# HKUST-Aerial-Robotics/ESVO

Measured on AMD Instinct MI355X. Metric: mapped events/sec (stereo TS raster + block matching + LM depth refinement + fusion), events resident in HBM before the timed region; exactly K ticks between two synchronisations, i.e. including the fill and the drain of the two-deep tick pipeline (`sustained`: the same workload over 1600 ticks), higher is better.
Workload: dtype f64

## Files before the change

esvo_amd/csrc/api_core.hip:

```cpp
#include "context.hpp"

namespace esvo_host {
thread_local std::string g_create_error;
}

namespace {

void invert3x3(const double* P, double* Kinv, double* Kinv_t) {
  const double a = P[0], b = P[1], cc = P[2], d = P[4], e = P[5], f = P[6], g = P[8], hh = P[9], i = P[10];
  const double det = a * (e * i - f * hh) - b * (d * i - f * g) + cc * (d * hh - e * g);
  const double id = 1.0 / det;
  Kinv[0] = (e * i - f * hh) * id; Kinv[1] = (cc * hh - b * i) * id; Kinv[2] = (b * f - cc * e) * id;
  Kinv[3] = (f * g - d * i) * id;  Kinv[4] = (a * i - cc * g) * id;  Kinv[5] = (cc * d - a * f) * id;
  Kinv[6] = (d * hh - e * g) * id; Kinv[7] = (b * g - a * hh) * id;  Kinv[8] = (a * e - b * d) * id;
  for (int r = 0; r < 3; ++r) Kinv_t[r] = (Kinv[r * 3 + 0] * P[3] + Kinv[r * 3 + 1] * P[7]) + Kinv[r * 3 + 2] * P[11];
}

int validate_params(const esvo_params_t* p, std::string& why) {
  if (p->ls_norm != ESVO_LSNORM_TDIST && p->ls_norm != ESVO_LSNORM_L2) { why = "LSnorm must be Tdist or l2 (DepthProblemSolver.cpp:121-131 exits on anything else)"; return ESVO_ERR_UNSUPPORTED; }
  if (p->bm_step < 1) { why = "BM_step must be >= 1"; return ESVO_ERR_INVALID_ARG; }
  if (p->patch_size_x < 1 || p->patch_size_x > 64 || p->patch_size_y < 1 || p->patch_size_y > 40) { why = "patch size must be within 1..64 x 1..40"; return ESVO_ERR_UNSUPPORTED; }
  if (p->median_blur_kernel_size < 0 || p->median_blur_kernel_size > 3) { why = "median_blur_kernel_size must be 0..3 (kernel 2k + 1)"; return ESVO_ERR_UNSUPPORTED; }
  if (p->max_event_queue_len < 0 || p->max_event_queue_len > TSQ_LMAX) { why = "max_event_queue_len must be 0 (one stamp per pixel) or 1..32"; return ESVO_ERR_UNSUPPORTED; }
  if (p->bm_max_disparity < p->bm_min_disparity || p->bm_min_disparity < 0) { why = "bad disparity range"; return ESVO_ERR_INVALID_ARG; }
// ... 194 lines not shown
  h->ring_cap = (u64)std::max<int64_t>(params->event_ring_capacity, 1024);
  for (int cam = 0; cam < 2; ++cam) CK(dalloc(&h->d_ring[cam], h->ring_cap));
  h->max_poses = (u32)std::max(params->max_poses_per_tick, 2);
  CK(dalloc(&h->d_pose_T2[0], (size_t)h->max_poses * 17));
  CK(dalloc(&h->d_pose_T2[1], (size_t)h->max_poses * 17));
  h->d_pose_T = h->d_pose_T2[0];
  h->max_ev = (u32)std::max(params->max_events_per_tick, params->process_event_num) + 1u;
  if (h->max_ev > 4000000u) { g_create_error = "max_events_per_tick too large (scan limit 4M)"; esvo_destroy(h); return ESVO_ERR_CAPACITY; }
  if (npx > 4000000u) { g_create_error = "image too large (scan limit 4M pixels)"; esvo_destroy(h); return ESVO_ERR_CAPACITY; }
  const size_t E = h->max_ev;
  CK(dalloc(&h->d_tick_ev, E));
  CK(dalloc(&h->d_match_slots, E));
  CK(dalloc(&h->d_match_flags, E));
  CK(dalloc(&h->d_match_prefix, E));
  CK(dalloc(&h->d_matches2[0], E));
  CK(dalloc(&h->d_matches2[1], E));
  h->d_matches = h->d_matches2[0];
  if (E >= LM_SPLIT_MIN_EVENTS) {
    CK(dalloc(&h->d_lm_fvec0, E * 7 * 16));
    CK(dalloc(&h->d_lm_fnorm0, E));
    CK(dalloc(&h->d_lm_meta, E));
    CK(dalloc(&h->d_lm_order, E));
    CK(dalloc(&h->d_lm_hist, 2 * 32 * 64));
    CK(hipMemset(h->d_lm_hist, 0, sizeof(u32) * 2 * 32 * 64));
  }
  if (E > LM_TWO_QUEUES_MAX_EVENTS) {
    for (int k = 0; k < 2; ++k) {
      CK(dalloc(&h->d_lm_pix_order2[k], E));
      CK(dalloc(&h->d_lm_sort_rows[k], E));
    }
    CK(dalloc(&h->d_lm_sort_hist, voxel_hist_words(E)));
    if (const char* eo = esvo_dev_switch("ESVO_LM_ORDER")) h->lm_order_on = std::atoi(eo) != 0;
  }
  CK(dalloc(&h->d_clk, 2 * clk_words(h->max_ev)));
  CK(hipMemset(h->d_clk, 0, sizeof(u64) * 2 * clk_words(h->max_ev)));
  if (const char* ec = esvo_dev_switch("ESVO_CLK_PROBE")) h->clk_probe = std::atoi(ec) != 0;
  {
    int khz = 0;
    if (hipDeviceGetAttribute(&khz, hipDeviceAttributeWallClockRate, device) != hipSuccess || khz <= 0) khz = 100000;
    h->stats.clk_ref_khz = (uint32_t)khz;
  }
  for (int k = 0; k < 2; ++k) {
    CK(dalloc(&h->d_pt_slots2[k], E));
    CK(dalloc(&h->d_pt_flags2[k], E));
    CK(dalloc(&h->d_pt_prefix2[k], E));
    CK(dalloc(&h->d_scan_tmp_l2[k], scan_scratch_elems(std::max(E, npx)) + 8));
  }
  h->d_pt_slots = h->d_pt_slots2[0]; h->d_pt_flags = h->d_pt_flags2[0]; h->d_pt_prefix = h->d_pt_prefix2[0];
  h->d_scan_tmp_l = h->d_scan_tmp_l2[0];
  CK(dalloc(&h->d_pts_tmp, E));
  CK(dalloc(&h->d_stage[0], E));
  CK(dalloc(&h->d_stage[1], E));
  CK(dalloc(&h->d_counters2[0], CNT_ROW));
  CK(dalloc(&h->d_counters2[1], CNT_ROW));
  CK(hipMemset(h->d_counters2[0], 0, sizeof(u32) * CNT_ROW));
  CK(hipMemset(h->d_counters2[1], 0, sizeof(u32) * CNT_ROW));
  h->d_counters = h->d_counters2[0];
  CK(hipHostMalloc(reinterpret_cast<void**>(&h->h_counters), sizeof(u32) * CNT_ROW * 2));
  std::memset(h->h_counters, 0, sizeof(u32) * CNT_ROW * 2);
  CK(hipHostMalloc(reinterpret_cast<void**>(&h->h_pin), sizeof(double) * 2 * ((size_t)h->max_poses * 17 + 16)));
  CK(dalloc(&h->d_scan_tmp, scan_scratch_elems(std::max(E, npx)) + 8));
  CK(dalloc(&h->d_scan_tmp_b, scan_scratch_elems(std::max(E, npx)) + 8));
  CK(dalloc(&h->d_cnt_b, CNTB_ROW));
  CK(hipMemset(h->d_cnt_b, 0, sizeof(u32) * CNTB_ROW));
  CK(hipHostMalloc(reinterpret_cast<void**>(&h->h_cnt_b), sizeof(u32) * CNTB_ROW * CNTB_ROWS));
  std::memset(h->h_cnt_b, 0, sizeof(u32) * CNTB_ROW * CNTB_ROWS);
// ... 50 lines not shown
  CK(dalloc(&h->d_export_cell, npx));
  for (int i = 0; i < EV_N; ++i) CK(hipEventCreate(&h->evt[i]));
  if (h->tl_on) { CK(hipEventCreate(&h->tl_ref)); CK(hipEventRecord(h->tl_ref, h->stream)); CK(hipEventSynchronize(h->tl_ref)); }
  h->evt_ok = true;
  CK(hipEventCreateWithFlags(&h->evt_trk_read, hipEventDisableTiming));
  for (int cam = 0; cam < 2; ++cam) CK(hipEventCreateWithFlags(&h->evt_ingest[cam], hipEventDisableTiming));
  CK(hipHostMalloc(reinterpret_cast<void**>(&h->h_pose_pool), sizeof(double) * 16 * (size_t)h->max_poses * esvo_context::POSE_POOL));
  for (int i = 0; i < esvo_context::POSE_POOL; ++i) CK(hipEventCreate(&h->pool_evt[i]));
  h->pool_ok = true;
  for (int i = 0; i < 16; ++i) h->T_world_obs[i] = h->T_world_frame[i] = (i % 5 == 0) ? 1.0 : 0.0;
#undef CK
  *out = h;
  return ESVO_OK;
}

int esvo_destroy(esvo_handle h) {
  if (!h) return ESVO_OK;
  hipSetDevice(h->device);
  if (h->stream) hipStreamSynchronize(h->stream);
  if (h->stream_l) hipStreamSynchronize(h->stream_l);
  if (h->stream_l1) hipStreamSynchronize(h->stream_l1);
  if (h->stream_b) hipStreamSynchronize(h->stream_b);
  comm_release(h);
  em_release(h);
  gpc_release(h);
  void* ptrs[] = {h->d_lut, h->d_mask, h->d_fixmap[0], h->d_fixmap[1], h->d_sae[0], h->d_sae[1], h->d_raw, h->d_raw1, h->d_fwd_lut[0], h->d_fwd_lut[1], h->d_fwd_off[0], h->d_fwd_off[1],
                  h->d_fwd_src[0], h->d_fwd_src[1], h->d_fwd_val, h->d_ts[0],
                  h->d_ts[1], h->d_ring[0], h->d_ring[1], h->d_obs2[0][0], h->d_obs2[0][1], h->d_obs2[1][0], h->d_obs2[1][1], h->d_obs_tmp,
                  h->d_pose_T2[0], h->d_pose_T2[1], h->d_scan_tmp_b, h->d_cnt_b, h->d_tick_ev, h->d_match_slots, h->d_match_flags, h->d_match_prefix,
                  h->d_matches2[0], h->d_matches2[1], h->d_scan_tmp_l2[0], h->d_scan_tmp_l2[1], h->d_pt_slots2[0], h->d_pt_slots2[1], h->d_pt_flags2[0], h->d_pt_flags2[1], h->d_pt_prefix2[0], h->d_pt_prefix2[1], h->d_pts_tmp, h->d_stage[0], h->d_stage[1], h->d_counters2[0], h->d_counters2[1], h->d_scan_tmp,
                  h->d_win, h->d_frame_pose_T, h->d_fr_table, h->d_prop, h->d_tile_pts, h->d_tile_count, h->d_over_pts,
                  h->d_cell_count, h->d_cell_offset, h->d_cell_list, h->d_fuse_ctr, h->d_rec_ids, h->d_map, h->d_map2, h->d_owner_max, h->d_owner_min, h->d_exp_flags,
                  h->d_exp_prefix, h->d_export, h->d_export_cell, h->d_reg_ab, h->d_reg_cd, h->d_tsq[0], h->d_tsq[1], h->d_tsq_tcount, h->d_tsq_tlist, h->d_tsq_over, h->d_tsq_over_count, h->d_own_w, h->d_lkeep, h->d_codes, h->d_codes_send, h->d_codes_all, h->d_pts_send, h->d_pts_all, h->d_rank_kept,
                  h->d_sel, h->d_evmap, h->d_lm_fvec0, h->d_lm_fnorm0, h->d_lm_meta, h->d_lm_order, h->d_lm_hist, h->d_lm_pix_order2[0], h->d_lm_pix_order2[1], h->d_lm_sort_rows[0], h->d_lm_sort_rows[1], h->d_lm_sort_hist, h->d_clk, h->d_ring_gidx, h->d_halo_viol, h->d_dn_flags, h->d_merge_a, h->d_merge_b, h->d_merge_plan, h->d_tsq_dup};
  for (void* p : ptrs) if (p) hipFree(p);
  if (h->h_counters) hipHostFree(h->h_counters);
  if (h->h_cnt_b) hipHostFree(h->h_cnt_b);
  if (h->h_pin) hipHostFree(h->h_pin);
  if (h->h_fr_table) hipHostFree(h->h_fr_table);
  if (h->evt_ok) for (int i = 0; i < EV_N; ++i) hipEventDestroy(h->evt[i]);
  if (h->pool_ok) for (int i = 0; i < esvo_context::POSE_POOL; ++i) hipEventDestroy(h->pool_evt[i]);
  if (h->h_pose_pool) hipHostFree(h->h_pose_pool);
  if (h->h_trk_ne) hipHostFree(h->h_trk_ne);
  if (h->h_trk_solve) hipHostFree(h->h_trk_solve);
  if (h->h_trk_xyz) hipHostFree(h->h_trk_xyz);
  release_routing(h);
  for (int cam = 0; cam < 2; ++cam) if (h->d_wire[cam]) hipFree(h->d_wire[cam]);
  if (h->evt_trk_read) hipEventDestroy(h->evt_trk_read);
  for (void* q : {(void*)h->d_cloud_xyz[0], (void*)h->d_cloud_xyz[1], (void*)h->d_cloud_ids, (void*)h->d_cloud_scan, (void*)h->d_cloud_cnt}) if (q) hipFree(q);
  if (h->h_cloud_cnt) hipHostFree(h->h_cloud_cnt);
  for (int k = 0; k < 2; ++k) {
    if (h->evt_cloud_built[k]) hipEventDestroy(h->evt_cloud_built[k]);
    if (h->evt_cloud_read[k]) hipEventDestroy(h->evt_cloud_read[k]);
  }
  if (h->tl_ref) hipEventDestroy(h->tl_ref);
  for (int cam = 0; cam < 2; ++cam) if (h->evt_ingest[cam]) hipEventDestroy(h->evt_ingest[cam]);
  for (void* q : {(void*)h->d_viz_bgr, (void*)h->d_viz_jet, (void*)h->d_viz_owner}) if (q) hipFree(q);
  for (void* q : {(void*)h->sgm.sobL, (void*)h->sgm.rawL, (void*)h->sgm.sobR, (void*)h->sgm.rawR, (void*)h->sgm.vol[0], (void*)h->sgm.vol[1],
                  (void*)h->sgm.vol[2], (void*)h->sgm.vol[3], (void*)h->sgm.vol[4], (void*)h->sgm.vol[5], (void*)h->sgm.d1, (void*)h->sgm.d1b,
                  (void*)h->sgm.d2key, (void*)h->d_sgm_img[0], (void*)h->d_sgm_img[1], (void*)h->d_sgm_disp, (void*)h->d_sgm_pair, (void*)h->d_sgm_T})
    if (q) hipFree(q);
  for (hipEvent_t e : h->evt_sgm) if (e) hipEventDestroy(e);
  if (h->own_stream && h->stream) hipStreamDestroy(h->stream);
  if (h->stream_b) hipStreamDestroy(h->stream_b);
  if (h->stream_l) { hipStreamSynchronize(h->stream_l); hipStreamDestroy(h->stream_l); }
  if (h->stream_l1) { hipStreamSynchronize(h->stream_l1); hipStreamDestroy(h->stream_l1); }
  if (h->stream_t) { hipStreamSynchronize(h->stream_t); hipStreamDestroy(h->stream_t); }
// ... 240 lines not shown
```

esvo_amd/csrc/api_dev.hip:

```cpp
#include <vector>

#include "context.hpp"
#include "fdiv.hpp"

namespace {
using esvo::u32;

constexpr size_t GUARD_WORDS = 64;
constexpr size_t GUARD_BYTES = GUARD_WORDS * sizeof(u32);
constexpr u32 GUARD_PATTERN = 0xA55AC33Cu;

struct GBuf {
  uint8_t* base = nullptr;
  size_t bytes = 0;
  bool pinned = false;
  GBuf() = default;
  GBuf(const GBuf&) = delete;
  GBuf& operator=(const GBuf&) = delete;
  ~GBuf() {
    if (!base) return;
    if (pinned) hipHostFree(base);
    else hipFree(base);
  }
  hipError_t make(size_t n, const void* init, bool pin = false) {
// ... 336 lines not shown
    hipLaunchKernelGGL(debug_recip_kernel, dim3(fdiv_blocks(n)), dim3(256), 0, st.s, d_b.ptr<double>(), n, d_m.ptr<double>(),
                       d_r.ptr<double>());
  DEV_RUN_DONE();
  HIPCHK(d_m.finish(y_make, &bad));
  HIPCHK(d_r.finish(y_refined, &bad));
  DEV_RETURN();
}

int esvo_debug_sqrt_moderate(const double* x, size_t n, double* out) {
  if (n && (!x || !out)) return ESVO_ERR_INVALID_ARG;
  DEV_BEGIN();
  GBuf d_x, d_out;
  HIPCHK(d_x.make(n * 8, x));
  HIPCHK(d_out.make(n * 8, out));
  if (n) hipLaunchKernelGGL(debug_sqrt_kernel, dim3(fdiv_blocks(n)), dim3(256), 0, st.s, d_x.ptr<double>(), n, d_out.ptr<double>());
  DEV_RUN_DONE();
  HIPCHK(d_out.finish(out, &bad));
  DEV_RETURN();
}

int esvo_debug_fuse_cell_counts(esvo_handle h, uint32_t* out, size_t n) {
  if (!h || !out) return ESVO_ERR_INVALID_ARG;
  API_LOCK(h);
  if (n != (size_t)h->W * (size_t)h->H) FAIL(ESVO_ERR_INVALID_ARG, "esvo_debug_fuse_cell_counts: width x height words are expected");
  HIPCHK(hipSetDevice(h->device));
  int rc = flush_pending_tick(h);
  if (rc) return rc;
  rc = drain_lm_and_back(h);
  if (rc) return rc;
  HIPCHK(hipMemcpy(out, h->d_cell_count, sizeof(u32) * n, hipMemcpyDeviceToHost));
  return ESVO_OK;
}

}
```

esvo_amd/csrc/api_map.hip:

```cpp
#include "context.hpp"

namespace esvo_host {

u64 lower_bound_sec(const esvo_context* h, int cam, double t) {
  const auto& v = h->ts_host[cam];
  size_t lo = 0, hi = v.size();
  while (lo < hi) {
    size_t mid = (lo + hi) / 2;
    if (ns_to_sec(v[mid]) < t) lo = mid + 1; else hi = mid;
  }
  return h->ring_base[cam] + lo;
}
u64 ros_time_from_sec(double t) {
  long long sec64 = (long long)std::floor(t);
  u32 sec = (u32)sec64;
  u32 nsec = (u32)std::round((t - sec) * 1e9);
  sec += (nsec / 1000000000ul);
  nsec %= 1000000000ul;
  return (u64)sec * 1000000000ull + nsec;
}

int upload_poses(esvo_context* h, const uint64_t* pose_t_ns, const double* pose_T, size_t m, u32* d_zero_row) {
  if (m > h->max_poses) FAIL(ESVO_ERR_CAPACITY, "pose table larger than max_poses_per_tick");
  h->pin_slot ^= 1;
  double* pin = h->h_pin + (size_t)h->pin_slot * ((size_t)h->max_poses * 17 + 16);
  double* T = pin;
  double* sec = pin + 16 * m;
  for (size_t i = 0; i < m; ++i) sec[i] = ns_to_sec(pose_t_ns[i]);
  std::memcpy(T, pose_T, sizeof(double) * 16 * m);
  h->h_pose_T.assign(pose_T, pose_T + 16 * m);
  h->n_pose = (u32)m;
  h->pose_buf ^= 1;
  h->d_pose_T = h->d_pose_T2[h->pose_buf];
  HIPCHK(hipStreamWaitEvent(h->stream, h->evt[EV_POSE + h->pose_buf * EV_BACK_STRIDE], 0));
  h->d_pose_sec = h->d_pose_T + 16 * m;
  launch_upload_words(T, h->d_pose_T, sizeof(double) * 17 * m, h->stream, d_zero_row, CNT_ROW);
  return ESVO_OK;
}

int run_bm(esvo_context* h, const esvo_event_t* d_ev, u64 first, u64 cap, int reverse, u32 n, const u32* sel) {
  BmArgs a;
  a.ev = d_ev; a.n = n; a.ev_first = first; a.ev_cap = cap; a.ev_reverse = reverse; a.sel = sel;
  a.tsL = h->d_obs[0]; a.tsR = h->d_obs[1];
  a.lut = h->d_lut; a.mask = h->d_mask;
  a.pose_sec = h->d_pose_sec; a.n_pose = h->n_pose;
  a.out_slots = h->d_match_slots; a.out_flags = h->d_match_flags;
  a.fail_counters = h->d_counters;
  if (h->stage_events_on) hipEventRecord(h->evt[EV_BM0 + h->fpar * EV_FRONT_STRIDE], h->stream);
  launch_bm_match(a, h->dp, h->stream);
  if (h->stage_events_on) hipEventRecord(h->evt[EV_BM1 + h->fpar * EV_FRONT_STRIDE], h->stream);
  HIPCHK(hipGetLastError());
  return ESVO_OK;
}
int run_order_matches(esvo_context* h, u32 n, bool local, bool by_index) {
  if (scan_compact_is_small(n)) {
    by_index = by_index && !local;
    launch_scan_compact_matches_small(h->d_match_flags, h->d_match_prefix, h->d_counters + (local ? CNT_OWN_MATCHES : CNT_MATCHES), n, h->d_match_slots,
                                      by_index ? nullptr : h->d_matches, (local || by_index) ? h->d_own_w : nullptr, h->stream);
  } else {
    launch_exclusive_scan_u32(h->d_match_flags, h->d_match_prefix, h->d_counters + (local ? CNT_OWN_MATCHES : CNT_MATCHES), h->d_scan_tmp, n, h->stream);
    launch_compact_matches(h->d_match_slots, h->d_match_flags, h->d_match_prefix, n, h->d_matches, local ? h->d_own_w : nullptr,
                           h->stream);
  }
  if (h->stage_events_on) hipEventRecord(h->evt[EV_S1 + h->fpar * EV_FRONT_STRIDE], h->stream);
  HIPCHK(hipGetLastError());
  return ESVO_OK;
}
int run_match(esvo_context* h, const esvo_event_t* d_ev, u64 first, u64 cap, int reverse, u32 n) {
  int rc = run_bm(h, d_ev, first, cap, reverse, n);
  if (rc) return rc;
  return run_order_matches(h, n, false);
}

void switch_front_parity(esvo_context* h) {
  h->fpar ^= 1;
  h->d_matches = h->d_matches2[h->fpar];
  h->d_counters = h->d_counters2[h->fpar];
  h->d_pt_slots = h->d_pt_slots2[h->fpar]; h->d_pt_flags = h->d_pt_flags2[h->fpar]; h->d_pt_prefix = h->d_pt_prefix2[h->fpar];
  h->d_scan_tmp_l = h->d_scan_tmp_l2[h->fpar];
}
static int lm_pair_policy(esvo_context* h, u32 n_events) {
  if (n_events == 0 || n_events > esvo::LM_PAIR_MAX_EVENTS || h->prm.ls_norm == ESVO_LSNORM_L2) return -1;
// ... 576 lines not shown
```

esvo_amd/csrc/common.hpp:

```cpp
#pragma once

#include <hip/hip_runtime.h>
#include <stdint.h>

#include "../../include/esvo_hip.h"

#define ESVO_WAVE 64

#include <cstdlib>
#include <cstring>
inline const char* esvo_dev_switch(const char* name) {
  const char* on = std::getenv("ESVO_DEV_SWITCHES");
  return (on && std::strcmp(on, "1") == 0) ? std::getenv(name) : nullptr;
}

namespace esvo {

typedef unsigned long long u64;
typedef unsigned int u32;

struct CamConst {
  double P[12];
  double Kinv[9];
  double Kinv_t[3];
// ... 166 lines not shown
                              uint8_t* d_raw, uint8_t* d_out, int W, int H, u64 t_ns, double decay_sec, int ignore_polarity,
                              int median_k, hipStream_t s);
void launch_gaussian5_pair(const uint8_t* in0, const uint8_t* in1, uint8_t* out0, uint8_t* out1, int W, int H, hipStream_t s,
                           int row0 = 0, int row1 = -1);
void launch_denoise_flags(const esvo_event_t* ring, u64 first, u64 cap, u32 n, uint8_t* evmap, u32* flags, int W, int H,
                          hipStream_t s);
void launch_denoise_select(const u32* flags, const u32* prefix, u32 n, u32* sel, hipStream_t s);
void launch_denoise_bits_routed(const esvo_event_t* ring, u64 first, u64 cap, u32 n_loc, const u32* gidx, u32 g_first, u32 n, uint8_t* evmap,
                                int W, int H, int band_y0, int band_y1, u32* bits, hipStream_t s);
void launch_denoise_bits_unpack(const u32* blocks, u32 block_words, u32 N, u32 n, u32* flags, hipStream_t s);

struct BmArgs {
  const esvo_event_t* ev;
  u32 n;
  u64 ev_first;
  u64 ev_cap;
  int ev_reverse;
  const u32* sel;
  const uint8_t* tsL;
  const uint8_t* tsR;
  const float2* lut;
  const uint8_t* mask;
  const double* pose_sec;
  u32 n_pose;
  esvo_match_t* out_slots;
  u32* out_flags;
  u32* fail_counters;
  const u32* gidx = nullptr;
  u32 g_first = 0;
  u32 n_loc = 0;
  const u32* keep_flags = nullptr;
  const u32* keep_prefix = nullptr;
  u32 n_raw = 0;
};
void launch_bm_match(const BmArgs& a, const DevParams& p, hipStream_t s);
void launch_compact_matches(const esvo_match_t* slots, const u32* flags, const u32* prefix, u32 n,
                            esvo_match_t* out, u32* slot_of, hipStream_t s);
void launch_matches_to_points(const esvo_match_t* m, const u32* n_ptr, u32 max_n, esvo_depth_point_t* out, const DevParams& p,
                              hipStream_t s);

struct TrackRef { double T[16]; };
struct TrackPose { double T[16]; double Jc[6]; };
#define TRK_NE_MAX_POSES 4
struct TrackPoseSet { TrackPose p[TRK_NE_MAX_POSES]; };
struct TrackArgs {
  const double* pts;
  const uint8_t* neg;
  const int16_t* du;
  const int16_t* dv;
  const uint8_t* mask;
  double P[12];
  int W, H;
};
void launch_track_images(const uint8_t* blurred, uint8_t* neg, int16_t* du, int16_t* dv, int W, int H, hipStream_t s);
void launch_track_reference(const float* xyz, u32 n, const TrackRef& r, double* pts, hipStream_t s);
void launch_track_reference_gather(const float* cloud_xyz, const u32* order, u32 n, const TrackRef& r, double* pts, hipStream_t s);
void launch_track_residuals(const TrackArgs& a, const TrackPose& pose, u32 offset, u32 count, int huber, double thr, double* fvec,
                            hipStream_t s);
void launch_track_jacobian(const TrackArgs& a, const TrackPose& pose, u32 offset, u32 count, double* fjac, hipStream_t s);
#define TRK_NE_THREADS 256
#define TRK_NE_TERMS 28
void launch_track_normal(const TrackArgs& a, const TrackPoseSet& poses, int n_poses, u32 offset, u32 count, int huber, double thr,
                         double* out28_per_pose, hipStream_t s);
#define TRK_SOLVE_MAX_ITERATIONS 64
#define TRK_SOLVE_THREADS 1024
struct TrackSolveArgs {
  double R0[9], t0[3];
  double huber_threshold, damping;
// ... 152 lines not shown
```

esvo_amd/csrc/context.hpp:

```cpp
#pragma once
#include <algorithm>
#include <array>
#include <atomic>
#include <chrono>
#include <cmath>
#include <cstdio>
#include <cstdlib>
#include <cstring>
#include <deque>
#include <mutex>
#include <string>
#include <vector>

#include "common.hpp"

using namespace esvo;

enum { EV_SC0 = 0, EV_SC1, EV_R1, EV_SC0b, EV_SC1b, EV_R1b, EV_FRAME,
       EV_T0, EV_BM0, EV_BM1, EV_S1, EV_LM0, EV_LM1, EV_S2, EV_CNT, EV_STG, EV_A1, EV_T0b, EV_BM0b, EV_BM1b, EV_S1b, EV_LM0b, EV_LM1b, EV_S2b, EV_CNTb, EV_STGb, EV_A1b,
       EV_FU0, EV_FU1, EV_CL1, EV_RG1, EV_POSE, EV_FU0b, EV_FU1b, EV_CL1b, EV_RG1b, EV_POSEb, EV_N };
constexpr int EV_BACK_STRIDE = EV_FU0b - EV_FU0;
constexpr int EV_FRONT_STRIDE = EV_T0b - EV_T0;
constexpr int EV_TS_STRIDE = EV_SC0b - EV_SC0;

// ... 90 lines not shown
  bool ingest_pending[2] = {false, false};

  uint8_t* d_obs[2] = {nullptr, nullptr};
  uint8_t* d_obs_tmp = nullptr;
  double T_world_obs[16];
  u64 obs_t_ns = 0;
  bool obs_set = false;

  double* d_pose_sec = nullptr;
  double* d_pose_T = nullptr;
  double* d_pose_T2[2] = {nullptr, nullptr};
  int pose_buf = 0;
  std::vector<double> h_pose_T;
  double* h_pin = nullptr;
  int pin_slot = 0;
  bool stats_pending = false;
  u32 n_pose = 0;

  u32 max_ev = 0;
  esvo_event_t* d_tick_ev = nullptr;
  esvo_match_t* d_match_slots = nullptr;
  u32* d_match_flags = nullptr;
  u32* d_match_prefix = nullptr;
  esvo_match_t* d_matches = nullptr;
  double* d_lm_fvec0 = nullptr;
  double* d_lm_fnorm0 = nullptr;
  u32* d_lm_meta = nullptr;
  u32* d_lm_order = nullptr;
  u32* d_lm_hist = nullptr;
  u32* d_lm_pix_order2[2] = {nullptr, nullptr};
  u64* d_lm_sort_rows[2] = {nullptr, nullptr};
  u32* d_lm_sort_hist = nullptr;
  bool lm_order_on = true;
  u64* d_clk = nullptr;
  bool clk_probe = true;
  DevPoint* d_pt_slots = nullptr;
  u32* d_pt_flags = nullptr;
  u32* d_pt_prefix = nullptr;
  DevPoint* d_pt_slots2[2] = {nullptr, nullptr};
  u32* d_pt_flags2[2] = {nullptr, nullptr};
  u32* d_pt_prefix2[2] = {nullptr, nullptr};
  DevPoint* d_pts_tmp = nullptr;
  DevPoint* d_stage[2] = {nullptr, nullptr};
  u32* d_counters = nullptr;
  u32* h_counters = nullptr;
  u32* d_scan_tmp = nullptr;
  u32* d_cnt_b = nullptr;
  u32* h_cnt_b = nullptr;
  u32* d_scan_tmp_b = nullptr;

  DevPoint* d_win = nullptr;
  u32 win_cap = 0;
  std::deque<FrameRec> frames;
  u32 n_pose_slots = 0;
  std::vector<char> slot_used;
  double* d_frame_pose_T = nullptr;
  u32 max_poses = 0;
  u32* d_fr_table = nullptr;
  u32* h_fr_table = nullptr;
  u32 max_frames = 0;
  size_t n_window_frames = 0;

  DevPoint* d_prop = nullptr;
  u32* d_tile_count = nullptr;
  uint2* d_tile_pts = nullptr;
  uint2* d_over_pts = nullptr;
// ... 279 lines not shown
```

esvo_amd/csrc/kernels_bm.hip:

```cpp
#include "common.hpp"
#include "fdiv.hpp"

namespace esvo {

__device__ inline int wave_sum_i32(int v) {
#pragma unroll
  for (int d = 32; d >= 1; d >>= 1) v += __shfl_xor(v, d, ESVO_WAVE);
  return v;
}
__device__ inline long long wave_sum_i64(long long v) {
#pragma unroll
  for (int d = 32; d >= 1; d >>= 1) v += __shfl_xor(v, d, ESVO_WAVE);
  return v;
}

typedef u32 u32x4_a4 __attribute__((ext_vector_type(4), aligned(4)));

struct ZnccLeft {
  double sigl;
  int Sl;
};
__device__ inline double sqrt_var(double v) { return v > 0 ? sqrt_moderate(v) : 0.0; }
__device__ inline ZnccLeft zncc_left(int Sl, int Sll, int N, const Recip& rn2) {
  ZnccLeft z;
// ... 42 lines not shown
  wv.w = __builtin_amdgcn_alignbyte(d[4], d[3], sh) & 0x00ffffffu;
  return wv;
}

__device__ inline void bm_item(const BmArgs& a, const DevParams& p, u32 w, u32& k, uint4& e, bool& ok) {
  if (a.gidx) {
    const u64 ei = (a.ev_first - w) % a.ev_cap;
    e = reinterpret_cast<const uint4*>(a.ev)[ei];
    k = a.g_first - a.gidx[ei];
    if (a.keep_flags) {
      ok = k < a.n_raw && a.keep_flags[k] != 0u;
      if (ok) k = a.keep_prefix[k];
      return;
    }
    ok = k < a.n;
    return;
  }
  k = stride_item(w, a.n, (u32)p.num_threads);
  const u32 kk = a.sel ? a.sel[k] : k;
  const u64 ei = (a.ev_reverse ? (a.ev_first - kk) : (a.ev_first + kk)) % a.ev_cap;
  e = reinterpret_cast<const uint4*>(a.ev)[ei];
}

template <int G>
__device__ inline void grp_argmin(double& best, int& bestd) {
#pragma unroll
  for (int s = G / 2; s >= 1; s >>= 1) {
    const double oc = __shfl_xor(best, s, G);
    const int od = __shfl_xor(bestd, s, G);
    if (od >= 0 && (bestd < 0 || oc < best || (oc == best && od > bestd))) { best = oc; bestd = od; }
  }
}

template <int G, bool COARSE, bool UPDOWN>
__global__ void __launch_bounds__(BM_BLOCK) bm_match_kernel(BmArgs a, DevParams p, int RD, int lds_per_event) {
  constexpr int EPB = BM_BLOCK / G;
  const int grp = threadIdx.x / G, l = threadIdx.x % G;
  const u32 pos = blockIdx.x * EPB + grp;
  const u32 w = a.gidx ? pos : pos * (u32)p.ev_nshards + (u32)p.ev_shard;
  const u32 n_out = a.gidx ? a.n_loc : a.n;
  u32* ldsL = reinterpret_cast<u32*>(bm_smem + grp * lds_per_event);
  u32* ldsR = ldsL + 28;
  const int nd = p.dmax - p.dmin + 1;
  double* cost_row = reinterpret_cast<double*>(ldsR + (UPDOWN ? (nd + 6) * 4 : 7 * RD));

  const int W = p.W, H = p.H;
  constexpr int wx = 15, wy = 7, N = wx * wy, hx = 7, hy = 3;

  bool ok = w < n_out;
  u32 k = 0;
  uint4 e = make_uint4(0, 0, 0, 0);
  if (ok) bm_item(a, p, w, k, e, ok);
  const int ex = e.x & 0xffffu, ey = e.x >> 16;
  double xr = 0, yr = 0;
  int x1 = 0, y1 = 0;
  if (ok) ok = ex < W && ey < H;
  if (ok) {
    const float2 q = a.lut[ey * W + ex];
    xr = (double)q.x;
    yr = (double)q.y;
    ok = !(xr < 0 || xr > (double)(W - 1) || yr < 0 || yr > (double)(H - 1));
    if (a.gidx && ok) { const int yb = (int)floor(yr); ok = yb >= p.band_y0 && yb < p.band_y1; }
  }
  if (ok && a.mask) ok = a.mask[(int)yr * W + (int)xr] > 125;
  if (ok) {
    x1 = (int)floor(xr);
    y1 = (int)floor(yr);
  }
  if (ok) ok = !(x1 - hx < 1 || y1 - hy < 1 || x1 + hx >= W - 1 || y1 + hy >= H - 1);
  int reason = 0;

  int Sl = 0, Sll = 0;
  if (ok) {
// ... 121 lines not shown
    __syncthreads();
    if (ok) {
      const int step = p.step;
      const int nc = (p.dmax - p.dmin) / step + 1;
      for (int j = l; j < nc; j += G) {
        const int d = p.dmin + j * step;
        if (!cand_valid(d)) continue;
        const double c = cost_row[d - p.dmin];
        if (c <= best) { best = c; bestd = d; }
      }
      grp_argmin<G>(best, bestd);
      bool found = bestd >= 0 && bestd - step >= p.dmin && bestd + step <= p.dmin + (nc - 1) * step;
      if (found) found = cost_row[bestd - step - p.dmin] < 1.0 && cost_row[bestd + step - p.dmin] < 1.0 && best < p.zncc_thr;
      if (!found) { ok = false; reason = 2; }
      else {
        const int cd = bestd;
        double fb = 2.0;
        int fd = -1;
        for (int d = cd - (step - 1) + l; d <= cd + (step - 1); d += G) {
          if (!cand_valid(d)) continue;
          const double c = cost_row[d - p.dmin];
          if (c <= fb) { fb = c; fd = d; }
        }
        grp_argmin<G>(fb, fd);
        best = fb;
        bestd = fd;
        if (!(best < p.zncc_thr)) { ok = false; reason = 3; }
      }
    }
  } else if (ok) {
    grp_argmin<G>(best, bestd);
    if (!(bestd >= 0 && best < p.zncc_thr)) { ok = false; reason = 2; }
  }
  u32 pose_idx = 0;
  if (ok) {
    const double te = time_to_sec(e.y, e.z);
    u32 lo = 0, hi = a.n_pose;
    while (lo < hi) {
      const u32 mid = (lo + hi) >> 1;
      if (a.pose_sec[mid] < te) lo = mid + 1; else hi = mid;
    }
    pose_idx = lo;
    ok = lo < a.n_pose;
  }
  if (w < n_out && l == 0) {
    a.out_flags[w] = ok ? 1u : 0u;
    if (ok) {
      esvo_match_t m;
      const double disparity = (double)bestd;
      const double depth = p.baseline_f / disparity;
      m.x_left[0] = xr;
      m.x_left[1] = yr;
      m.inv_depth = 1.0 / depth;
      m.cost = best;
      m.disp = disparity;
      m.event_idx = k;
      m.pose_idx = pose_idx;
      a.out_slots[w] = m;
    }
  }
  if (a.fail_counters) {
    const bool lead = w < n_out && l == 0;
#pragma unroll
    for (int r = 1; r <= 3; ++r) {
      const int n = __popcll(__ballot(lead && reason == r));
      if (n && (threadIdx.x & 63) == 0)
        atomicAdd(a.fail_counters + CNT_BM_FAIL + (r - 1) * CNT_STRIPES + (blockIdx.x % CNT_STRIPES), (u32)n);
    }
  }
}

__device__ inline double zncc_any(long long Sl, long long Sll, long long Sr, long long Srr, long long Slr, int N) {
  const double n = (double)N;
  const double varl = (double)(N * Sll - Sl * Sl) / (n * n);
  const double varr = (double)(N * Srr - Sr * Sr) / (n * n);
  const double sigl = sqrt(varl) + 1e-6, sigr = sqrt(varr) + 1e-6;
  const double cov = (double)(N * Slr - Sl * Sr) / n;
  return 0.5 * (1 - cov / (sigl * sigr) / n);
}
__device__ inline uint8_t ts_byte_clamped(const uint8_t* ts, int n_px, int idx) {
// ... 183 lines not shown
}
template <bool COARSE, bool UPDOWN>
static void launch_bm_mode(int G, const BmArgs& a, const DevParams& p, int RD, hipStream_t s) {
  switch (G) {
    case 64: launch_bm_g<64, COARSE, UPDOWN>(a, p, RD, s); break;
    case 32: launch_bm_g<32, COARSE, UPDOWN>(a, p, RD, s); break;
    case 16: launch_bm_g<16, COARSE, UPDOWN>(a, p, RD, s); break;
    default: launch_bm_g<8, COARSE, UPDOWN>(a, p, RD, s); break;
  }
}

void launch_bm_match(const BmArgs& a, const DevParams& p, hipStream_t s) {
  if (a.n == 0) return;
  const int nd = p.dmax - p.dmin + 1;
  const int RD = ((((nd + 2) >> 2) + 5) + 3) & ~3;
  int bestG = 64, bestSlots = 1 << 30;
  for (int G = 64; G >= 8; G >>= 1) {
    const int slots = ((nd + G - 1) / G) * G;
    if (slots < bestSlots) { bestSlots = slots; bestG = G; }
  }
  const bool coarse = p.step > 1;
  if (p.wx != 15 || p.wy != 7) {
    if (p.updown) { if (coarse) launch_bm_any<true, true>(a, p, s); else launch_bm_any<false, true>(a, p, s); }
    else { if (coarse) launch_bm_any<true, false>(a, p, s); else launch_bm_any<false, false>(a, p, s); }
    return;
  }
  if (p.updown) {
    if (coarse) launch_bm_mode<true, true>(bestG, a, p, RD, s);
    else launch_bm_mode<false, true>(bestG, a, p, RD, s);
  } else {
    if (coarse) launch_bm_mode<true, false>(bestG, a, p, RD, s);
    else launch_bm_mode<false, false>(bestG, a, p, RD, s);
  }
}

__global__ void __launch_bounds__(256) compact_matches_kernel(const esvo_match_t* __restrict__ slots, const u32* __restrict__ flags,
                                                              const u32* __restrict__ prefix, u32 n,
                                                              esvo_match_t* __restrict__ out, u32* __restrict__ slot_of) {
  const u32 w = blockIdx.x * blockDim.x + threadIdx.x;
  if (w >= n || !flags[w]) return;
  out[prefix[w]] = slots[w];
  if (slot_of) slot_of[prefix[w]] = w;
}
void launch_compact_matches(const esvo_match_t* slots, const u32* flags, const u32* prefix, u32 n, esvo_match_t* out,
                            u32* slot_of, hipStream_t s) {
  if (n == 0) return;
  hipLaunchKernelGGL(compact_matches_kernel, dim3((n + 255) / 256), dim3(256), 0, s, slots, flags, prefix, n, out, slot_of);
}

__global__ void __launch_bounds__(256) matches_to_points_kernel(const esvo_match_t* __restrict__ m, const u32* __restrict__ n_ptr,
                                                                u32 max_n, DevPoint* __restrict__ out, DevParams p) {
  const u32 i = blockIdx.x * blockDim.x + threadIdx.x;
  u32 n = *n_ptr;
  if (n > max_n) n = max_n;
  if (i >= n) return;
  const esvo_match_t e = m[i];
  DevPoint o;
  o.row = (u32)(size_t)floor(e.x_left[1]);
  o.col = (u32)(size_t)floor(e.x_left[0]);
  o.x[0] = e.x_left[0];
  o.x[1] = e.x_left[1];
  cam2World(p.camL, e.x_left[0], e.x_left[1], e.inv_depth, o.p_cam);
  o.inv_depth = e.inv_depth;
  o.variance = 1e-6;
  o.scale2 = 0;
  o.nu = 0;
// ... 13 lines not shown
```

esvo_amd/lib.py:

```python
import ctypes as C
import os
import subprocess

import numpy as np

from .abi import (DEPTH_POINT_DTYPE, EM_POSE_FN, ERR_CAPACITY, ERR_INVALID_ARG, ERR_STATE, EVENT_DTYPE, MATCH_DTYPE, CalibStruct, EmSelectionStruct,
                  EmStatsStruct, GpcParamsStruct, GpcStatsStruct, ParamsStruct, SgmStatsStruct, StatsStruct, TRACK_ITER_DTYPE, TRACK_SOLVE_MAX_ITERATIONS,
                  TrackSolveInfoStruct, TrackSolveParamsStruct)

_CSRC = os.path.join(os.path.dirname(os.path.abspath(__file__)), "csrc")
_LIB_PATH = os.environ.get("ESVO_HIP_LIB") or os.path.join(_CSRC, "libesvo_hip.so")
_SOURCES = ["api_core.hip", "api_ts.hip", "api_map.hip", "api_window.hip", "api_modes.hip", "api_shard.hip", "api_out.hip", "api_comm.hip", "api_bag.hip", "api_track.hip", "scan.hip", "kernels_ts.hip", "kernels_bm.hip", "kernels_lm.hip", "kernels_lm_any.hip", "kernels_fuse.hip", "kernels_shard.hip", "kernels_track.hip", "kernels_track_viz.hip", "kernels_viz.hip", "kernels_sgm.hip", "api_em.hip", "kernels_em.hip", "kernels_cloud.hip", "api_dev.hip", "api_gpc.hip", "kernels_voxel.hip"]
HIPCC_FLAGS = ["--offload-arch=gfx950", "-O3", "-std=c++17", "-ffp-contract=off", "-fPIC", "-shared",
               "-Wno-unused-value", "-Wno-unused-result", "-ldl"]

SYMBOLS = [
    "esvo_default_params", "esvo_create", "esvo_destroy", "esvo_reset", "esvo_set_params", "esvo_last_error",
    "esvo_set_stream", "esvo_synchronize", "esvo_ts_push_events", "esvo_ts_push_events_async", "esvo_ts_push_wait", "esvo_host_alloc", "esvo_host_free", "esvo_ts_push_event_array", "esvo_ts_render", "esvo_ts_render_forward", "esvo_map_set_observation",
    "esvo_map_match", "esvo_map_set_poses", "esvo_map_refine", "esvo_map_push_frame", "esvo_map_fuse",
    "esvo_map_tick", "esvo_map_tick_bm_only", "esvo_map_fuse_matches_naive", "esvo_map_tick_resident", "esvo_map_get_depth_points", "esvo_map_get_committed", "esvo_map_get_pointcloud_xyz", "esvo_map_get_last_frame",
    "esvo_get_stats", "esvo_shard_set_band", "esvo_shard_set_routing", "esvo_shard_get_rows", "esvo_shard_exchange", "esvo_shard_tick_phase", "esvo_abi_sizes",
    "esvo_map_front", "esvo_map_front_frame", "esvo_map_push_frame_device", "esvo_map_fuse_async",
    "esvo_track_set_current", "esvo_track_get_images", "esvo_track_set_reference", "esvo_track_residuals", "esvo_track_jacobian",
    "esvo_track_normal_equations", "esvo_track_normal_equations_batch", "esvo_track_register", "esvo_track_solve", "esvo_track_sizes",
# ... 746 lines not shown
        return int(n.value), disp

    def push_disparity_frame(self, disp16, ev):
        d = None if disp16 is None else np.ascontiguousarray(disp16, np.int16)
        assert d is None or d.shape == (self.H, self.W)
        ev = np.ascontiguousarray(ev, dtype=EVENT_DTYPE)
        n = C.c_size_t()
        self._ck(self.lib.esvo_map_push_disparity_frame(self.h, _p(d), ev.ctypes.data if len(ev) else None, ev.shape[0], C.byref(n)))
        return int(n.value)

    def sgm_stats(self):
        s = SgmStatsStruct()
        self._ck(self.lib.esvo_map_sgm_stats(self.h, C.byref(s)))
        return s

    def tick_resident(self, t_ns, T_world_cam, stamps, poses):
        st = np.ascontiguousarray(stamps, np.uint64)
        T = np.ascontiguousarray(poses, np.float64).reshape(-1, 16)
        Tw = np.ascontiguousarray(T_world_cam, np.float64).reshape(16)
        self._ck(self.lib.esvo_map_tick_resident(self.h, int(t_ns), Tw.ctypes.data, st.ctypes.data, T.ctypes.data, st.shape[0]))

    def get_map(self):
        n = C.c_size_t(0)
        out = np.zeros(self.W * self.H, DEPTH_POINT_DTYPE)
        self._ck(self.lib.esvo_map_get_depth_points(self.h, out.ctypes.data, out.shape[0], C.byref(n)))
        return out[: n.value].copy()

    def debug_fuse_cell_counts(self):
        out = np.zeros((self.H, self.W), np.uint32)
        fn = _dbg_fn("esvo_debug_fuse_cell_counts", [C.c_void_p, C.c_void_p, C.c_size_t])
        self._ck(fn(self.h, out.ctypes.data, out.size))
        return out

    def get_committed_map(self):
        out = np.zeros(self.W * self.H, DEPTH_POINT_DTYPE)
        n, t = C.c_size_t(), C.c_uint64()
        self._ck(self.lib.esvo_map_get_committed(self.h, out.ctypes.data, out.shape[0], C.byref(n), C.byref(t)))
        return out[:n.value].copy(), int(t.value)

    def get_pointcloud(self):
        n = C.c_size_t(0)
        out = np.zeros((self.W * self.H, 3), np.float32)
        self._ck(self.lib.esvo_map_get_pointcloud_xyz(self.h, out.ctypes.data, out.shape[0], C.byref(n)))
        return out[: n.value].copy()

    def map_cloud_build(self):
        n = C.c_size_t(0)
        self._ck(self.lib.esvo_map_cloud_build(self.h, C.byref(n)))
        return int(n.value)

    def map_cloud(self):
        n = C.c_size_t(0)
        self._ck(self.lib.esvo_map_cloud_get(self.h, None, 0, C.byref(n)))
        out = np.zeros((int(n.value), 3), np.float32)
        if n.value:
            self._ck(self.lib.esvo_map_cloud_get(self.h, out.ctypes.data, out.shape[0], C.byref(n)))
        return out

    def map_cloud_device(self):
        ptr, n, t = C.c_void_p(), C.c_size_t(), C.c_uint64()
        self._ck(self.lib.esvo_map_cloud_device(self.h, C.byref(ptr), C.byref(n), C.byref(t)))
        return (ptr.value or 0), int(n.value), int(t.value)

    def get_debug_images(self, age_max_range=10.0):
        imgs = [np.empty((self.H, self.W, 3), np.uint8) for _ in range(4)]
        self._ck(self.lib.esvo_map_get_debug_images(self.h, float(age_max_range), *[i.ctypes.data for i in imgs]))
# ... 277 lines not shown
```

Before: 175.1 million.

## Deduplicate block-matching searches for events sharing a pixel

```diff
diff --git a/esvo_amd/csrc/api_core.hip b/esvo_amd/csrc/api_core.hip
--- a/esvo_amd/csrc/api_core.hip
+++ b/esvo_amd/csrc/api_core.hip
@@ -250,6 +250,9 @@
     CK(dalloc(&h->d_lm_sort_hist, voxel_hist_words(E)));
     if (const char* eo = esvo_dev_switch("ESVO_LM_ORDER")) h->lm_order_on = std::atoi(eo) != 0;
   }
+  if (const char* ed = esvo_dev_switch("ESVO_BM_DEDUPE")) h->bm_dedupe_on = std::atoi(ed) != 0;
+  if (const char* em = esvo_dev_switch("ESVO_BM_DEDUPE_MIN")) h->bm_dedupe_min = (u32)std::max(1L, std::atol(em));
+  if (h->bm_dedupe_on && E >= h->bm_dedupe_min) CK(dalloc(&h->d_bm_dedupe, npx + 4 + 2 * E));
   CK(dalloc(&h->d_clk, 2 * clk_words(h->max_ev)));
   CK(hipMemset(h->d_clk, 0, sizeof(u64) * 2 * clk_words(h->max_ev)));
   if (const char* ec = esvo_dev_switch("ESVO_CLK_PROBE")) h->clk_probe = std::atoi(ec) != 0;
@@ -366,7 +369,7 @@
                   h->d_win, h->d_frame_pose_T, h->d_fr_table, h->d_prop, h->d_tile_pts, h->d_tile_count, h->d_over_pts,
                   h->d_cell_count, h->d_cell_offset, h->d_cell_list, h->d_fuse_ctr, h->d_rec_ids, h->d_map, h->d_map2, h->d_owner_max, h->d_owner_min, h->d_exp_flags,
                   h->d_exp_prefix, h->d_export, h->d_export_cell, h->d_reg_ab, h->d_reg_cd, h->d_tsq[0], h->d_tsq[1], h->d_tsq_tcount, h->d_tsq_tlist, h->d_tsq_over, h->d_tsq_over_count, h->d_own_w, h->d_lkeep, h->d_codes, h->d_codes_send, h->d_codes_all, h->d_pts_send, h->d_pts_all, h->d_rank_kept,
-                  h->d_sel, h->d_evmap, h->d_lm_fvec0, h->d_lm_fnorm0, h->d_lm_meta, h->d_lm_order, h->d_lm_hist, h->d_lm_pix_order2[0], h->d_lm_pix_order2[1], h->d_lm_sort_rows[0], h->d_lm_sort_rows[1], h->d_lm_sort_hist, h->d_clk, h->d_ring_gidx, h->d_halo_viol, h->d_dn_flags, h->d_merge_a, h->d_merge_b, h->d_merge_plan, h->d_tsq_dup};
+                  h->d_sel, h->d_evmap, h->d_lm_fvec0, h->d_lm_fnorm0, h->d_lm_meta, h->d_lm_order, h->d_lm_hist, h->d_lm_pix_order2[0], h->d_lm_pix_order2[1], h->d_lm_sort_rows[0], h->d_lm_sort_rows[1], h->d_lm_sort_hist, h->d_bm_dedupe, h->d_clk, h->d_ring_gidx, h->d_halo_viol, h->d_dn_flags, h->d_merge_a, h->d_merge_b, h->d_merge_plan, h->d_tsq_dup};
   for (void* p : ptrs) if (p) hipFree(p);
   if (h->h_counters) hipHostFree(h->h_counters);
   if (h->h_cnt_b) hipHostFree(h->h_cnt_b);
diff --git a/esvo_amd/csrc/api_dev.hip b/esvo_amd/csrc/api_dev.hip
--- a/esvo_amd/csrc/api_dev.hip
+++ b/esvo_amd/csrc/api_dev.hip
@@ -392,4 +392,18 @@
   return ESVO_OK;
 }
 
-}
+int esvo_debug_bm_owner_count(esvo_handle h, uint32_t* n_owners, int* shared) {
+  if (!h || !n_owners || !shared) return ESVO_ERR_INVALID_ARG;
+  API_LOCK(h);
+  HIPCHK(hipSetDevice(h->device));
+  int rc = flush_pending_tick(h);
+  if (rc) return rc;
+  *n_owners = 0;
+  *shared = h->d_bm_dedupe ? 1 : 0;
+  if (!h->d_bm_dedupe) return ESVO_OK;
+  HIPCHK(hipStreamSynchronize(h->stream));
+  HIPCHK(hipMemcpy(n_owners, h->d_bm_dedupe + (size_t)h->W * h->H, sizeof(u32), hipMemcpyDeviceToHost));
+  return ESVO_OK;
+}
+
+}
diff --git a/esvo_amd/csrc/api_map.hip b/esvo_amd/csrc/api_map.hip
--- a/esvo_amd/csrc/api_map.hip
+++ b/esvo_amd/csrc/api_map.hip
@@ -47,7 +47,14 @@
   a.out_slots = h->d_match_slots; a.out_flags = h->d_match_flags;
   a.fail_counters = h->d_counters;
   if (h->stage_events_on) hipEventRecord(h->evt[EV_BM0 + h->fpar * EV_FRONT_STRIDE], h->stream);
-  launch_bm_match(a, h->dp, h->stream);
+  if (h->d_bm_dedupe && n >= h->bm_dedupe_min && n <= h->max_ev && !h->sharded && bm_dedupe_applies(a, h->dp)) {
+    u32* owner = h->d_bm_dedupe;
+    u32* n_uniq = owner + (size_t)h->W * h->H;
+    u32* uniq_w = n_uniq + 4;
+    launch_bm_match_dedupe(a, h->dp, owner, uniq_w, n_uniq, uniq_w + h->max_ev, h->stream);
+  } else {
+    launch_bm_match(a, h->dp, h->stream);
+  }
   if (h->stage_events_on) hipEventRecord(h->evt[EV_BM1 + h->fpar * EV_FRONT_STRIDE], h->stream);
   HIPCHK(hipGetLastError());
   return ESVO_OK;
diff --git a/esvo_amd/csrc/common.hpp b/esvo_amd/csrc/common.hpp
--- a/esvo_amd/csrc/common.hpp
+++ b/esvo_amd/csrc/common.hpp
@@ -222,8 +222,14 @@
   const u32* keep_flags = nullptr;
   const u32* keep_prefix = nullptr;
   u32 n_raw = 0;
+  const u32* uniq_w = nullptr;
+  const u32* n_uniq = nullptr;
+  u32* search_rec = nullptr;
 };
 void launch_bm_match(const BmArgs& a, const DevParams& p, hipStream_t s);
+constexpr u32 BM_DEDUPE_MIN_EVENTS = 40001u;
+bool bm_dedupe_applies(const BmArgs& a, const DevParams& p);
+void launch_bm_match_dedupe(BmArgs a, const DevParams& p, u32* owner, u32* uniq_w, u32* n_uniq, u32* search_rec, hipStream_t s);
 void launch_compact_matches(const esvo_match_t* slots, const u32* flags, const u32* prefix, u32 n,
                             esvo_match_t* out, u32* slot_of, hipStream_t s);
 void launch_matches_to_points(const esvo_match_t* m, const u32* n_ptr, u32 max_n, esvo_depth_point_t* out, const DevParams& p,
diff --git a/esvo_amd/csrc/context.hpp b/esvo_amd/csrc/context.hpp
--- a/esvo_amd/csrc/context.hpp
+++ b/esvo_amd/csrc/context.hpp
@@ -146,6 +146,9 @@
   u64* d_lm_sort_rows[2] = {nullptr, nullptr};
   u32* d_lm_sort_hist = nullptr;
   bool lm_order_on = true;
+  u32* d_bm_dedupe = nullptr;
+  bool bm_dedupe_on = true;
+  u32 bm_dedupe_min = esvo::BM_DEDUPE_MIN_EVENTS;
   u64* d_clk = nullptr;
   bool clk_probe = true;
   DevPoint* d_pt_slots = nullptr;
diff --git a/esvo_amd/csrc/kernels_bm.hip b/esvo_amd/csrc/kernels_bm.hip
--- a/esvo_amd/csrc/kernels_bm.hip
+++ b/esvo_amd/csrc/kernels_bm.hip
@@ -98,13 +98,28 @@
   }
 }
 
+__device__ inline u32 pose_lower_bound(const BmArgs& a, const uint4& e) {
+  const double te = time_to_sec(e.y, e.z);
+  u32 lo = 0, hi = a.n_pose;
+  while (lo < hi) {
+    const u32 mid = (lo + hi) >> 1;
+    if (a.pose_sec[mid] < te) lo = mid + 1; else hi = mid;
+  }
+  return lo;
+}
+
 template <int G, bool COARSE, bool UPDOWN>
 __global__ void __launch_bounds__(BM_BLOCK) bm_match_kernel(BmArgs a, DevParams p, int RD, int lds_per_event) {
   constexpr int EPB = BM_BLOCK / G;
   const int grp = threadIdx.x / G, l = threadIdx.x % G;
   const u32 pos = blockIdx.x * EPB + grp;
-  const u32 w = a.gidx ? pos : pos * (u32)p.ev_nshards + (u32)p.ev_shard;
   const u32 n_out = a.gidx ? a.n_loc : a.n;
+  u32 w = a.gidx ? pos : pos * (u32)p.ev_nshards + (u32)p.ev_shard;
+  if (a.uniq_w) {
+    const u32 nu = *a.n_uniq;
+    if (blockIdx.x * EPB >= nu) return;
+    w = pos < nu ? a.uniq_w[pos] : n_out;
+  }
   u32* ldsL = reinterpret_cast<u32*>(bm_smem + grp * lds_per_event);
   u32* ldsR = ldsL + 28;
   const int nd = p.dmax - p.dmin + 1;
@@ -292,20 +307,16 @@
     grp_argmin<G>(best, bestd);
     if (!(bestd >= 0 && best < p.zncc_thr)) { ok = false; reason = 2; }
   }
+  const bool found = ok;
   u32 pose_idx = 0;
   if (ok) {
-    const double te = time_to_sec(e.y, e.z);
-    u32 lo = 0, hi = a.n_pose;
-    while (lo < hi) {
-      const u32 mid = (lo + hi) >> 1;
-      if (a.pose_sec[mid] < te) lo = mid + 1; else hi = mid;
-    }
-    pose_idx = lo;
-    ok = lo < a.n_pose;
+    pose_idx = pose_lower_bound(a, e);
+    ok = pose_idx < a.n_pose;
   }
   if (w < n_out && l == 0) {
     a.out_flags[w] = ok ? 1u : 0u;
-    if (ok) {
+    if (a.uniq_w) a.search_rec[w] = (found ? 1u : 0u) | ((u32)reason << 1);
+    if (ok || (a.uniq_w && found)) {
       esvo_match_t m;
       const double disparity = (double)bestd;
       const double depth = p.baseline_f / disparity;
@@ -555,6 +566,96 @@
     if (coarse) launch_bm_mode<true, false>(bestG, a, p, RD, s);
     else launch_bm_mode<false, false>(bestG, a, p, RD, s);
   }
+}
+
+__global__ void __launch_bounds__(256) bm_claim_kernel(BmArgs a, DevParams p, u32* __restrict__ owner, u32* __restrict__ n_uniq) {
+  const u32 w = blockIdx.x * blockDim.x + threadIdx.x;
+  if (w == 0) *n_uniq = 0u;
+  if (w >= a.n) return;
+  u32 k = 0;
+  uint4 e;
+  bool ok = true;
+  bm_item(a, p, w, k, e, ok);
+  const int ex = e.x & 0xffffu, ey = e.x >> 16;
+  if (ex < p.W && ey < p.H) atomicMin(owner + ey * p.W + ex, w);
+}
+__global__ void __launch_bounds__(256) bm_owner_list_kernel(BmArgs a, DevParams p, const u32* __restrict__ owner, u32* __restrict__ uniq_w,
+                                                            u32* __restrict__ n_uniq) {
+  __shared__ u32 wave_cnt[4];
+  __shared__ u32 base;
+  const u32 w = blockIdx.x * blockDim.x + threadIdx.x;
+  bool own = false;
+  if (w < a.n) {
+    u32 k = 0;
+    uint4 e;
+    bool ok = true;
+    bm_item(a, p, w, k, e, ok);
+    const int ex = e.x & 0xffffu, ey = e.x >> 16;
+    own = !(ex < p.W && ey < p.H) || owner[ey * p.W + ex] == w;
+  }
+  const u64 bal = __ballot(own);
+  const u32 lane = threadIdx.x & 63u, wv = threadIdx.x >> 6;
+  if (lane == 0) wave_cnt[wv] = (u32)__popcll(bal);
+  __syncthreads();
+  if (threadIdx.x == 0) {
+    const u32 total = wave_cnt[0] + wave_cnt[1] + wave_cnt[2] + wave_cnt[3];
+    base = total ? atomicAdd(n_uniq, total) : 0u;
+  }
+  __syncthreads();
+  if (!own) return;
+  u32 off = base + (u32)__popcll(bal & ((1ull << lane) - 1ull));
+  for (u32 i = 0; i < wv; ++i) off += wave_cnt[i];
+  uniq_w[off] = w;
+}
+__global__ void __launch_bounds__(256) bm_fanout_kernel(BmArgs a, DevParams p, const u32* __restrict__ owner) {
+  const u32 w = blockIdx.x * blockDim.x + threadIdx.x;
+  int reason = 0;
+  if (w < a.n) {
+    u32 k = 0;
+    uint4 e;
+    bool ok = true;
+    bm_item(a, p, w, k, e, ok);
+    const int ex = e.x & 0xffffu, ey = e.x >> 16;
+    const u32 o = (ex < p.W && ey < p.H) ? owner[ey * p.W + ex] : w;
+    if (o != w) {
+      const u32 rec = a.search_rec[o];
+      reason = (int)(rec >> 1);
+      ok = (rec & 1u) != 0u;
+      u32 pose_idx = 0;
+      if (ok) {
+        pose_idx = pose_lower_bound(a, e);
+        ok = pose_idx < a.n_pose;
+      }
+      a.out_flags[w] = ok ? 1u : 0u;
+      if (ok) {
+        esvo_match_t m = a.out_slots[o];
+        m.event_idx = k;
+        m.pose_idx = pose_idx;
+        a.out_slots[w] = m;
+      }
+    }
+  }
+  if (a.fail_counters) {
+#pragma unroll
+    for (int r = 1; r <= 3; ++r) {
+      const int n = __popcll(__ballot(reason == r));
+      if (n && (threadIdx.x & 63) == 0)
+        atomicAdd(a.fail_counters + CNT_BM_FAIL + (r - 1) * CNT_STRIPES + (blockIdx.x % CNT_STRIPES), (u32)n);
+    }
+  }
+}
+bool bm_dedupe_applies(const BmArgs& a, const DevParams& p) {
+  return a.n > 0 && !a.gidx && !a.keep_flags && p.ev_nshards == 1 && p.wx == 15 && p.wy == 7;
+}
+void launch_bm_match_dedupe(BmArgs a, const DevParams& p, u32* owner, u32* uniq_w, u32* n_uniq, u32* search_rec, hipStream_t s) {
+  if (a.n == 0) return;
+  const dim3 grid((a.n + 255) / 256), block(256);
+  hipMemsetAsync(owner, 0xff, sizeof(u32) * (size_t)p.W * (size_t)p.H, s);
+  hipLaunchKernelGGL(bm_claim_kernel, grid, block, 0, s, a, p, owner, n_uniq);
+  hipLaunchKernelGGL(bm_owner_list_kernel, grid, block, 0, s, a, p, owner, uniq_w, n_uniq);
+  a.uniq_w = uniq_w; a.n_uniq = n_uniq; a.search_rec = search_rec;
+  launch_bm_match(a, p, s);
+  hipLaunchKernelGGL(bm_fanout_kernel, grid, block, 0, s, a, p, owner);
 }
 
 __global__ void __launch_bounds__(256) compact_matches_kernel(const esvo_match_t* __restrict__ slots, const u32* __restrict__ flags,
diff --git a/esvo_amd/lib.py b/esvo_amd/lib.py
--- a/esvo_amd/lib.py
+++ b/esvo_amd/lib.py
@@ -802,6 +802,12 @@
         self._ck(fn(self.h, out.ctypes.data, out.size))
         return out
 
+    def debug_bm_owner_count(self):
+        n, shared = C.c_uint32(0), C.c_int(0)
+        fn = _dbg_fn("esvo_debug_bm_owner_count", [C.c_void_p, C.c_void_p, C.c_void_p])
+        self._ck(fn(self.h, C.byref(n), C.byref(shared)))
+        return int(n.value) if shared.value else None
+
     def get_committed_map(self):
         out = np.zeros(self.W * self.H, DEPTH_POINT_DTYPE)
         n, t = C.c_size_t(), C.c_uint64()
```

Result: faster. 186.1 million, median of 6 (+6.3%).
